# qingfengxia/FenicsSolver

Measured on AMD Instinct MI355X. Metric: DOF/s (assemble+CG solve to 1e-8) on 3D heat transfer, higher is better.
Workload: dtype f64

## Files before the change

fenicssolver_amd/csrc/fs_krylov.hip:

```cpp
#include "fs_common.h"
#include "fs_kernels.h"
#include <functional>
#include <chrono>
#include <string>
#include <unordered_map>
#include <math.h>
#include <stdlib.h>

#ifndef FS_BLOCK_ROUND
#define FS_BLOCK_ROUND 3
#endif

#include "fs_krylov_stream.inc"

#include "fs_krylov_dict.inc"

#define BOX_DC_AUX 2
#include "fs_box.h"
#include "fs_latmarch.h"
#include "fs_krylov_lattice.inc"

#include "fs_krylov_dict3.inc"

struct row_dict {
// ... 2058 lines not shown
                    hipLaunchKernelGGL(k_cg_update<true>, dim3(vgrid), dim3(FS_BLOCK), 0, s, n, k, k == max_iter ? 1 : 0, ws.partials.p, sgrid, ws.sums.p, ws.ctrl.p, ws.scal.p, ws.status.p, hist_p, ws.dinv.p, ws.z.p, ws.w.p, ws.p.p, ws.s.p, x->d.p, ws.r.p);
                } else {
                    FS_CHECK(fs_comm_sum_allreduce_dev(ws.partials.p, sgrid, 3, ws.sums.p, s));
                    if (sample) FS_HIP(hipEventRecord(ws.ev[n_samples][2], s));
                    hipLaunchKernelGGL(k_cg_update<false>, dim3(vgrid), dim3(FS_BLOCK), 0, s, n, k, k == max_iter ? 1 : 0, ws.partials.p, sgrid, ws.sums.p, ws.ctrl.p, ws.scal.p, ws.status.p, hist_p, ws.dinv.p, ws.z.p, ws.w.p, ws.p.p, ws.s.p, x->d.p, ws.r.p);
                }
                if (sample) {
                    FS_HIP(hipEventRecord(ws.ev[n_samples][3], s));
                    ++n_samples;
                }
            }
            FS_KERNEL_CHECK();
            n_launches += k - k_before;
            if (!mirrored) {
                FS_HIP(hipMemcpyAsync(ws.h_status + 4 * slot, ws.status.p, 4 * sizeof(int), hipMemcpyDeviceToHost, s));
                FS_HIP(hipEventRecord(ws.poll[slot], s));
                if (pending >= 0) {
                    FS_HIP(hipEventSynchronize(ws.poll[pending]));
                    if (ws.h_status[4 * pending] != 0) finished = true;
                }
                pending = slot;
                slot ^= 1;
            }
            if (k > max_iter) finished = true;
        }
        lap("iterations of the pass");
        if (sp->halo.begun) {
            FS_CHECK(fs_halo_end_dev(sp, s));
            sp->halo.begun = false;
        }
        if (red_stream) FS_HIP(hipStreamWaitEvent(s, ws.ev_red, 0));
        if (iteration_form & 1) {
            hipLaunchKernelGGL(k_cg_pair_flush, dim3(fs_grid_for(n / 2 + 1, FS_BLOCK, 2048)), dim3(FS_BLOCK), 0, s, n, ws.status.p, ws.scal.p, ws.z.p, ws.p.p, x->d.p);
            FS_KERNEL_CHECK();
        }
        FS_HIP(hipMemcpyAsync(ws.z.p, x->d.p, (size_t)n * sizeof(double), hipMemcpyDeviceToDevice, s));
        FS_CHECK(fs_halo_exchange_dev(sp, ws.z.p, s));
        launch_spmv<0>(A, ws.z.p, ws.w.p, nullptr, nullptr, nullptr, s, aval);
        if (ds) hipLaunchKernelGGL(k_residual_scaled, dim3(pgrid), dim3(FS_BLOCK), 0, s, ws.bhat.p, ws.w.p, ws.dvec.p, n, (double*)nullptr, ws.partials.p);
        else hipLaunchKernelGGL(k_residual, dim3(pgrid), dim3(FS_BLOCK), 0, s, b->d.p, ws.w.p, n, (double*)nullptr, ws.partials.p);
        FS_CHECK(fs_comm_sum_allreduce_dev(ws.partials.p, pgrid, 1, ws.sums.p + 5, s));
        FS_HIP(hipMemcpyAsync(ws.h_status + 12, ws.status.p, 4 * sizeof(int), hipMemcpyDeviceToHost, s));
        FS_HIP(hipMemcpyAsync(ws.h_vals, ws.sums.p, 8 * sizeof(double), hipMemcpyDeviceToHost, s));
        FS_HIP(hipMemcpyAsync(ws.h_vals + 8, ws.ctrl.p, 4 * sizeof(double), hipMemcpyDeviceToHost, s));
        FS_HIP(hipStreamSynchronize(s));
        if (fs_p2p_reduce_enabled()) FS_CHECK(fs_p2p_check(s));
        for (int q = 0; q < 4; ++q) h_status[q] = ws.h_status[12 + q];
        const int iters = h_status[1];
        total_iters += iters;
        for (int i = first_sample; i < n_samples; ++i) ws.sample_live[i] = ws.sample_iter[i] + ws.sample_span[i] - 1 < iters;
        if (ws.h_status[8] != 0) {
            fs_set_error("fs_krylov_solve: %d zero%s diagonal entries (Jacobi preconditioner undefined)", ws.h_status[8], ds ? " or negative" : "");
            return FS_ERR_NUMERIC;
        }
        const double* h_pass = ws.h_vals;
        const double* h_ctrl2 = ws.h_vals + 8;
        true_rr = h_pass[5];
        thresh = h_ctrl2[0];
        bb_host = h_ctrl2[1];
        ++n_pass;
        if (getenv("FS_KRYLOV_DEBUG"))
            fprintf(stderr, "[fs_krylov] pass %d: status %d, %d iterations (total %d), true ||r||^2 %.3e, threshold %.3e\n",
                    n_pass, h_status[0], h_status[1], total_iters, true_rr, thresh);
        const bool recurrence_converged = h_status[0] == 1;
        if (!recurrence_converged || true_rr <= thresh * 1.0201 || n_pass >= 8 || total_iters >= opts->max_iter) break;
        if (true_rr > 0.7 * prev_true_rr) break;
        prev_true_rr = true_rr;
        use_guess = true;
    }
    if (ds) {
        hipLaunchKernelGGL(k_pointwise_mul, dim3(fs_grid_for(n)), dim3(FS_BLOCK), 0, s, ws.dinv.p, x->d.p, n, x->d.p);
        FS_KERNEL_CHECK();
    }
    const int iters = total_iters;
    if (fs_rt().comm && getenv("FS_COMM_TIMING")) {
        double au, hu; long ac, hc;
        fs_comm_host_time(&au, &ac, &hu, &hc, true);
        fprintf(stderr, "[fs_krylov] host time inside RCCL enqueue calls: all-reduce %.1f us x %ld, grouped send/recv %.1f us x %ld; %d iterations in %.1f ms\n",
                ac ? au / ac : 0.0, ac, hc ? hu / hc : 0.0, hc, iters,
                std::chrono::duration<double, std::milli>(std::chrono::steady_clock::now() - t_begin).count());
    }
#ifdef FS_ITER_TIMING
    if (fused && getenv("FS_ITER_TIMING")) {
        std::vector<long long> h(8 * 4096);
        FS_HIP(hipMemcpyFromSymbol(h.data(), HIP_SYMBOL(g_iter_dbg), h.size() * sizeof(long long)));
        long long first = h[0], last = 0;
        for (int b = 0; b < igrid; ++b) { first = std::min(first, h[8 * b]); last = std::max(last, h[8 * b + 7]); }
        double mean[8] = {0}, mx[8] = {0};
        for (int b = 0; b < igrid; ++b)
            for (int k2 = 0; k2 < 8; ++k2) { const double v = (h[8 * b + k2] - first) * 0.01; mean[k2] += v / igrid; mx[k2] = std::max(mx[k2], v); }
        fprintf(stderr, "[iter timing, last launch, us from the first workgroup's start] span %.2f;", (last - first) * 0.01);
        for (int k2 = 0; k2 < 8; ++k2) fprintf(stderr, " s%d mean %.2f max %.2f;", k2, mean[k2], mx[k2]);
        fprintf(stderr, "\n");
        std::vector<int32_t> hi((size_t)sp->n_dict_items * 4);
        FS_CHECK(sp->dict_items.download(hi.data(), (int64_t)hi.size(), s));
        FS_HIP(hipStreamSynchronize(s));
        const int64_t n_chunks = (sp->n_dict_items + 3) / 4, per_xcd = (n_chunks + 7) >> 3;
        int cnt[2] = {0, 0};
        double gm[2][3] = {{0}}, gx[2][3] = {{0}};
        for (int b = 0; b < igrid; ++b) {
            int64_t cur = b, step = igrid, end = n_chunks;
            if (dict_map_xcd()) { cur = (b & 7) * per_xcd + (b >> 3); step = igrid >> 3; end = std::min<int64_t>(((b & 7) + 1) * per_xcd, n_chunks); }
            int e = 0;
            for (; cur < end; cur += step)
                for (int64_t q = 4 * cur; q < std::min<int64_t>(4 * cur + 4, sp->n_dict_items); ++q) e |= (hi[(size_t)q * 4 + 1] >> 16) & 1;
            ++cnt[e];
            for (int k2 = 0; k2 < 3; ++k2) { const double v = (h[8 * b + 5 + k2] - first) * 0.01; gm[e][k2] += v; gx[e][k2] = std::max(gx[e][k2], v); }
        }
        for (int e = 0; e < 2; ++e) {
            fprintf(stderr, "[iter timing] %d workgroups %s an edge item:", cnt[e], e ? "with" : "without");
            for (int k2 = 0; k2 < 3; ++k2) fprintf(stderr, " s%d mean %.2f max %.2f;", 5 + k2, cnt[e] ? gm[e][k2] / cnt[e] : 0.0, gx[e][k2]);
            fprintf(stderr, "\n");
        }
    }
#endif
    ws.last_hist.resize((size_t)iters + 1);
    FS_CHECK(ws.hist.download(ws.last_hist.data(), iters + 1, s));
    const auto t_end = std::chrono::steady_clock::now();

    if (stats) {
        memset(stats, 0, sizeof(*stats));
        const double bb = bb_host;
        stats->iterations = iters;
        stats->converged = h_status[0] == 2 ? -1 : (h_status[0] == 1 ? 1 : 0);
        stats->bnorm = sqrt(bb);
        stats->rel_residual = bb > 0.0 ? sqrt(ws.last_hist[iters] / bb) : 0.0;
        stats->true_rel_residual = bb > 0.0 ? sqrt(true_rr / bb) : sqrt(true_rr);
        stats->solve_ms = std::chrono::duration<double, std::milli>(t_end - t_begin).count();
        double t_spmv = 0.0, t_upd = 0.0;
        int cnt = 0;
        for (int i = 0; i < n_samples; ++i) {
            if (!ws.sample_live[i]) continue;
            float a = 0.f, c = 0.f;
            if (hipEventElapsedTime(&a, ws.ev[i][0], ws.ev[i][1]) != hipSuccess) break;
            if (hipEventElapsedTime(&c, ws.ev[i][2], ws.ev[i][3]) != hipSuccess) break;
            t_spmv += a / (float)ws.sample_span[i];
            t_upd += c;
            ++cnt;
        }
        if (cnt) {
            stats->spmv_ms = t_spmv / cnt;
            stats->update_ms = t_upd / cnt;
        }
        stats->spmv_bytes = sp->nnz_nodes * bs * bs * 12 + n * 20;
        stats->row_classes = g_dict.built_for ? g_dict.ncls : 0;
        stats->fused_iteration = fusedp_used ? 2 : (fused ? 1 : 0);
        stats->classes_kept = g_dict.built_for && g_dict.kept ? 1 : 0;
        stats->launches = n_launches;
        stats->product_kind = fused ? (BI ? 3 : 1) : g_last_product_kind;
        g_last_iteration_form = (fused || fusedp_used) ? iteration_form : 0;
        if (fused) stats->update_ms = 0.0;
    }
    if (h_status[0] == 2) {
        fs_set_error("fs_krylov_solve: %s breakdown at iteration %d (operator not SPD / rho = 0 / NaN)", bicg ? "BiCGStab" : "CG", iters);
        return FS_ERR_NUMERIC;
    }
    return FS_OK;
}

extern "C" int fs_last_iteration_form() { return g_last_iteration_form & 3; }
extern "C" int fs_last_iteration_guard() { return (g_last_iteration_form >> 2) & 3; }
void fs_krylov_set_history(const std::vector<double>& rr) { g_ws.last_hist = rr; }
void fs_set_last_product_kind(int kind) { g_last_product_kind = kind; }

extern "C" int fs_krylov_history(double* out, int capacity, int* count) {
    const int n = (int)g_ws.last_hist.size();
    if (count) *count = n;
    if (out)
        for (int i = 0; i < n && i < capacity; ++i) out[i] = g_ws.last_hist[i];
    return FS_OK;
}

void fs_krylov_preload() {
    hipFuncAttributes attr;
    (void)hipFuncGetAttributes(&attr, reinterpret_cast<const void*>(k_set_threshold));
    (void)hipGetLastError();
}
```

fenicssolver_amd/csrc/fs_krylov_dict.inc:

```

constexpr int FS_DICT_CAP = 8192;
constexpr int FS_DICT_MAX = 4096;
constexpr int FS_DICT_ITEM_ROWS = 126;
constexpr int FS_DICT_WHOLE_LDS_BYTES = 32 << 10;
constexpr int FS_DICT_LDS_BYTES = 64 << 10;
constexpr int FS_DICT_ITEMS_PER_WAVE = 4;
constexpr int FS_DICT3_RUNS = 4;
constexpr int FS_DICT_MAX_ROUNDS = 8;

struct dict_plan_round {
    int32_t start[8];
    uint8_t len[8];
    uint8_t pad[24];
};
static_assert(sizeof(dict_plan_round) == 64, "one 64-byte scalar load per round");
struct dict_plan_round12 {
    int32_t start[12];
    uint8_t len[12];
    uint8_t pad[4];
};
static_assert(sizeof(dict_plan_round12) == 64, "one 64-byte scalar load per round");
__host__ __device__ __forceinline__ int32_t dict_run_start(const dict_plan_round* __restrict__ pl, int NR, int g) {
    return reinterpret_cast<const int32_t*>(pl + g / NR)[g % NR];
}
// ... 207 lines not shown
            if (slot_d) dtab[id] = slot_d[slot];
        }
        id += used;
    }
}

__global__ void __launch_bounds__(FS_BLOCK) k_dict_finish(int64_t n_items, const int4* __restrict__ items, const dict_plan_round* __restrict__ plans,
                                                          const int64_t* __restrict__ slice_ptr, const int32_t* __restrict__ dia_ptr,
                                                          const int32_t* __restrict__ dia_off, const double* __restrict__ val, int nq, int64_t plane, int S, int RL,
                                                          const int32_t* __restrict__ slot2cls, const double* __restrict__ values,
                                                          const int32_t* __restrict__ nnz, const uint16_t* __restrict__ cls_slot,
                                                          uint16_t* __restrict__ cls, int* info, const double* __restrict__ sc = nullptr, int NR = 8,
                                                          const double* __restrict__ dvec = nullptr, const double* __restrict__ dtab = nullptr) {
    const int lane = threadIdx.x & 63;
    int64_t q = ((int64_t)blockIdx.x * blockDim.x + threadIdx.x) >> 6;
    const int64_t stride = ((int64_t)gridDim.x * blockDim.x) >> 6;
    int bad = 0, bad_d = 0, crowded = 0;
    for (; q < n_items; q += stride) {
        const int4 it = items[q];
        const int32_t first = it.x, nr = it.y & 0xffff;
        const dict_plan_round* __restrict__ pl = plans + it.z;
        const int n_runs = NR * it.w;
        int id2[2] = {-1, -1};
        for (int half = 0; half < 2; ++half) {
            const int i = half * 64 + lane;
            if (i >= nr) continue;
            const int32_t r = first + i;
            const int id = slot2cls[cls_slot[r]];
            cls[r] = (uint16_t)(id < 0 ? 0 : id);
            if (id < 0 || id >= FS_DICT_MAX) { ++bad; continue; }
            id2[half] = id;
            if (dvec) bad_d += __double_as_longlong(dvec[r]) != __double_as_longlong(dtab[id]);
            const double* __restrict__ dv = values + (int64_t)id * S;
            int nz = 0, diff = 0;
            const bool fits = dict_walk_row(r, slice_ptr, dia_ptr, dia_off, val, nq, plane, pl, n_runs, RL, [&](int slot, double v) {
                ++nz;
                diff += slot >= S || __double_as_longlong(v) != __double_as_longlong(dv[slot < S ? slot : 0]);
            }, sc, NR);
            bad += !fits || diff != 0 || nz != nnz[id];
        }
        int distinct = 0;
        unsigned long long m0 = __ballot(id2[0] >= 0), m1 = __ballot(id2[1] >= 0);
        while (m0 | m1) {
            const bool from0 = m0 != 0ull;
            const int src = __ffsll((long long)(from0 ? m0 : m1)) - 1;
            const int cv = __shfl(from0 ? id2[0] : id2[1], src, 64);
            m0 &= ~__ballot(id2[0] == cv);
            m1 &= ~__ballot(id2[1] == cv);
            ++distinct;
        }
        crowded = distinct > crowded ? distinct : crowded;
    }
    if (bad) atomicAdd(&info[2], bad);
    if (bad_d) atomicAdd(&info[4], bad_d);
    if (crowded && lane == 0 && crowded > __hip_atomic_load(&info[3], __ATOMIC_RELAXED, __HIP_MEMORY_SCOPE_AGENT)) atomicMax(&info[3], crowded);
}

__device__ __forceinline__ double fs_from_next_lane(double v) {
    const int lo = __builtin_amdgcn_update_dpp(0, __double2loint(v), 0x130, 0xf, 0xf, true);
    const int hi = __builtin_amdgcn_update_dpp(0, __double2hiint(v), 0x130, 0xf, 0xf, true);
    return __hiloint2double(hi, lo);
}

__device__ __forceinline__ void fs_fill_lds(double* __restrict__ lds, const double* __restrict__ g, int n) {
    typedef double v2d __attribute__((ext_vector_type(2)));
    const int n2 = n >> 1;
    const v2d* __restrict__ g2 = reinterpret_cast<const v2d*>(g);
    v2d* __restrict__ l2 = reinterpret_cast<v2d*>(lds);
    for (int base = 0; base < n2; base += 4 * FS_BLOCK) {
        v2d t[4];
#pragma unroll
        for (int u = 0; u < 4; ++u) {
            const int i = base + u * FS_BLOCK + (int)threadIdx.x;
            t[u] = g2[i < n2 ? i : n2 - 1];
        }
#pragma unroll
        for (int u = 0; u < 4; ++u) {
            const int i = base + u * FS_BLOCK + (int)threadIdx.x;
            if (i < n2) l2[i] = t[u];
        }
    }
}

__device__ __forceinline__ void fs_wave_copy_pairs(double* __restrict__ lds, const double* __restrict__ g, int n2, int lane) {
    typedef double v2d __attribute__((ext_vector_type(2)));
    const v2d* __restrict__ g2 = reinterpret_cast<const v2d*>(g);
    v2d* __restrict__ l2 = reinterpret_cast<v2d*>(lds);
    for (int base = 0; base < n2; base += 256) {
        v2d t[4];
#pragma unroll
        for (int u = 0; u < 4; ++u) {
            const int i = base + u * 64 + lane;
            t[u] = g2[i < n2 ? i : n2 - 1];
        }
#pragma unroll
        for (int u = 0; u < 4; ++u) {
            const int i = base + u * 64 + lane;
            if (i < n2) l2[i] = t[u];
        }
    }
}

template <int DOTS, bool LDSD, int RL, int NR = 8>
__global__ void __launch_bounds__(FS_BLOCK) k_dict_spmv(int64_t n_cols, int64_t n_items, const int4* __restrict__ items,
                                                        const dict_plan_round* __restrict__ plans, const uint16_t* __restrict__ cls,
                                                        const double* __restrict__ dict, int S, int C,
                                                        const double* __restrict__ x, double* __restrict__ y,
                                                        const double* __restrict__ rvec, double* __restrict__ partials,
                                                        int* __restrict__ status, int part_base, int part_stride, int bump, int map_xcd) {
    const int st0 = DOTS ? status[0] : 0;
    typedef double v2d __attribute__((ext_vector_type(2)));
    typedef double v2du __attribute__((ext_vector_type(2), aligned(8)));
    extern __shared__ __attribute__((aligned(16))) double sdict[];
    __shared__ double lds4[4];
    const int lane = threadIdx.x & 63;
    const int wave = threadIdx.x >> 6;
    double* __restrict__ wl = LDSD ? sdict : sdict + (int64_t)wave * C * S;
    if (LDSD) fs_fill_lds(sdict, dict, C * S);
    if (DOTS) {
        if (st0 != 0) return;
        if (bump && blockIdx.x == 0 && threadIdx.x == 0) status[2] += 1;
    }
    if (LDSD) __syncthreads();
    double d_rz = 0.0, d_wz = 0.0, d_rr = 0.0;
    constexpr int K = LDSD ? 1 : FS_DICT_ITEMS_PER_WAVE;
    const int64_t n_chunks = (n_items + 4 * K - 1) / (4 * K);
    const int32_t cmax = (int32_t)(n_cols - 1);
    chunk_iter it = xcd_chunks(n_chunks);
    if (!map_xcd) { it.cur = blockIdx.x; it.step = gridDim.x; it.end = n_chunks; }
    int tagv = -1, rr = 0;
    const unsigned long long cmask = C >= 64 ? ~0ull : ((1ull << C) - 1ull);
    for (; it.cur < it.end; it.cur += it.step)
    for (int kk = 0; kk < K; ++kk) {
        const int64_t q = (it.cur * 4 + wave) * K + kk;
        if (q >= n_items) break;
        const int4 ds = items[__builtin_amdgcn_readfirstlane((int)q)];
        const int32_t first = __builtin_amdgcn_readfirstlane(ds.x);
        const int nr = __builtin_amdgcn_readfirstlane(ds.y) & 0xffff;
        const int edge = __builtin_amdgcn_readfirstlane(ds.y) >> 16;
        const dict_plan_round* __restrict__ pl = plans + __builtin_amdgcn_readfirstlane(ds.z);
        const int rounds = __builtin_amdgcn_readfirstlane(ds.w);
        const int32_t r = first + 2 * lane;
        const bool ok0 = 2 * lane < nr, ok1 = 2 * lane + 1 < nr;
        v2d ri = {0.0, 0.0};
        if (DOTS && DOTS != 4) {
            if (ok1) ri = *reinterpret_cast<const v2du*>(&rvec[r]);
            else if (ok0) ri.x = rvec[r];
        }
        int c0 = -1, c1 = -1;
        if ((first & 1) == 0) {
            const uint32_t two = *reinterpret_cast<const uint32_t*>(&cls[r]);
            if (ok0) c0 = (int)(two & 0xffffu);
            if (ok1) c1 = (int)(two >> 16);
        } else {
            if (ok0) c0 = (int)cls[r];
            if (ok1) c1 = (int)cls[r + 1];
        }
        const double* __restrict__ xr = x + r;
        v2d A[NR];
        struct starts8 { int32_t v[NR]; };
        auto read_starts = [&](const dict_plan_round* __restrict__ p) {
            starts8 t;
#pragma unroll
            for (int j = 0; j < NR; ++j) t.v[j] = __builtin_amdgcn_readfirstlane(reinterpret_cast<const int32_t*>(p)[j]);
            return t;
        };
// ... 111 lines not shown
```

fenicssolver_amd/csrc/fs_krylov_iter.inc:

```

__global__ void k_set_threshold(const double* __restrict__ bb, double rtol, double atol, double* __restrict__ ctrl) {
    if (threadIdx.x == 0 && blockIdx.x == 0) {
        const double t = rtol * rtol * bb[0];
        ctrl[0] = fmax(t, atol * atol);
        ctrl[1] = bb[0];
    }
}
__global__ void k_set_iteration_limit(double* __restrict__ ctrl, int max_iter) {
    if (threadIdx.x == 0 && blockIdx.x == 0) ctrl[2] = (double)max_iter;
}

__device__ __forceinline__ bool cg_scalars_from(int iter, double gamma, double delta, double rho, double gamma_old, double alpha_old,
                                                 double& alpha, double& beta) {
    beta = 0.0;
    if (iter == 0) {
        alpha = gamma / delta;
    } else {
        beta = gamma / gamma_old;
        alpha = gamma / (delta - beta * gamma / alpha_old);
    }
    return (alpha > 0.0) && (alpha < 1e300) && (rho == rho);
}
__device__ __forceinline__ bool cg_scalars(int iter, double gamma, double delta, double rho, const double* __restrict__ scal,
                                            double& alpha, double& beta) {
// ... 285 lines not shown
    const bool first_trip = i + stride < n2;
    double2 wa0 = {0.0, 0.0}, wb0 = wa0, pa0 = wa0, sa0 = wa0, xa0 = wa0, ra0 = wa0, pb0 = wa0, sb0 = wa0, xb0 = wa0, rb0 = wa0;
    if (first_trip) {
        const int64_t j = i + stride;
        wa0 = io::ld(&w2[i]); wb0 = io::ld(&w2[j]);
        pa0 = io::ld(&p2[i]); sa0 = io::ld(&s2[i]); xa0 = io::ld(&x2[i]); ra0 = io::ld(&r2[i]);
        pb0 = io::ld(&p2[j]); sb0 = io::ld(&s2[j]); xb0 = io::ld(&x2[j]); rb0 = io::ld(&r2[j]);
    }
    if (st0 != 0) return;
    if (iter < 0) {
        iter = st2 - 1;
        check_only = iter >= (int)it_max ? 1 : 0;
    }
    double gamma, delta, rho;
    if (FUSED) {
        double sm[3];
        wg_sum_partials<3>(partials, npart, sm);
        gamma = sm[0]; delta = sm[1]; rho = sm[2];
    } else {
        gamma = sums[0]; delta = sums[1]; rho = sums[2];
    }
    const bool leader = blockIdx.x == 0 && threadIdx.x == 0;
    if (leader) hist[iter] = rho;
    auto stop = [&](int code) {
        if (leader) {
            status[1] = iter; status[0] = code;
            if (mirror) { fs_host_store(mirror + 1, iter); fs_host_store(mirror, code); }
        }
    };
    if (rho <= thresh) { stop(1); return; }
    if (check_only) { stop(3); return; }
    double beta, alpha;
    if (!cg_scalars_from(iter, gamma, delta, rho, ((iter - 1) & 1) ? sc_g1 : sc_g0, ((iter - 1) & 1) ? sc_a1 : sc_a0, alpha, beta)) { stop(2); return; }
    if (leader) {
        scal[2 * (iter & 1) + 0] = gamma;
        scal[2 * (iter & 1) + 1] = alpha;
        if (mirror) fs_host_store(mirror + 1, iter + 1);
    }
    bool prefetched = first_trip;
    for (; i + stride < n2; i += 2 * stride) {
        const int64_t j = i + stride;
        double2 wa, wb, pa, sa, xa, ra, pb, sb, xb, rb;
        if (prefetched) {
            wa = wa0; wb = wb0; pa = pa0; sa = sa0; xa = xa0; ra = ra0; pb = pb0; sb = sb0; xb = xb0; rb = rb0;
            prefetched = false;
        } else {
            wa = io::ld(&w2[i]); wb = io::ld(&w2[j]);
            pa = io::ld(&p2[i]); sa = io::ld(&s2[i]); xa = io::ld(&x2[i]); ra = io::ld(&r2[i]);
            pb = io::ld(&p2[j]); sb = io::ld(&s2[j]); xb = io::ld(&x2[j]); rb = io::ld(&r2[j]);
        }
        pa.x = ra.x + beta * pa.x;  pa.y = ra.y + beta * pa.y;
        pb.x = rb.x + beta * pb.x;  pb.y = rb.y + beta * pb.y;
        sa.x = wa.x + beta * sa.x;  sa.y = wa.y + beta * sa.y;
        sb.x = wb.x + beta * sb.x;  sb.y = wb.y + beta * sb.y;
        xa.x += alpha * pa.x;       xa.y += alpha * pa.y;
        xb.x += alpha * pb.x;       xb.y += alpha * pb.y;
        ra.x -= alpha * sa.x;       ra.y -= alpha * sa.y;
        rb.x -= alpha * sb.x;       rb.y -= alpha * sb.y;
        if (r_plain & 2) { p2[i] = pa; p2[j] = pb; } else { io::st(&p2[i], pa); io::st(&p2[j], pb); }
        if (r_plain & 4) { s2[i] = sa; s2[j] = sb; } else { io::st(&s2[i], sa); io::st(&s2[j], sb); }
        if (r_plain & 8) { x2[i] = xa; x2[j] = xb; } else { io::st(&x2[i], xa); io::st(&x2[j], xb); }
        if (r_plain & 1) { r2[i] = ra; r2[j] = rb; } else { io::st(&r2[i], ra); io::st(&r2[j], rb); }
    }
    for (; i < n2; i += stride) {
        const double2 ww = w2[i];
        double2 pp = p2[i], ss = s2[i], xx = x2[i], rr = r2[i];
        pp.x = rr.x + beta * pp.x;  pp.y = rr.y + beta * pp.y;
        ss.x = ww.x + beta * ss.x;  ss.y = ww.y + beta * ss.y;
        xx.x += alpha * pp.x;       xx.y += alpha * pp.y;
        rr.x -= alpha * ss.x;       rr.y -= alpha * ss.y;
        p2[i] = pp; s2[i] = ss; x2[i] = xx; r2[i] = rr;
    }
    if ((n & 1) && blockIdx.x == 0 && threadIdx.x == 0) {
        const int64_t t = n - 1;
        const double pp = r[t] + beta * p[t];
        const double ss = w[t] + beta * sv[t];
        p[t] = pp; sv[t] = ss;
        x[t] += alpha * pp;
        r[t] -= alpha * ss;
    }
}

#ifdef FS_ITER_TIMING
__device__ long long g_iter_dbg[8 * 4096];
#define FS_STAMP(k) do { if (threadIdx.x == 0 && it_ctr[par] == 100) g_iter_dbg[8 * blockIdx.x + (k)] = wall_clock64(); } while (0)
#else
#define FS_STAMP(k) do { } while (0)
#endif
enum { FS_ITER_EVERY = 0, FS_ITER_LIGHT = 1, FS_ITER_PAIR = 2 };
template <int RL, bool COMM, int MODE = FS_ITER_EVERY, bool DTAB = false, bool GUARD = false, bool CENTRE = false>
__global__ void __launch_bounds__(FS_BLOCK) k_dict_cg_iter(int64_t n_cols, int64_t n_items, const int4* __restrict__ items,
                                                           const dict_plan_round* __restrict__ plans, const uint16_t* __restrict__ cls,
                                                           const double* __restrict__ dict, int S, int C,
                                                           const double* __restrict__ r_in, const double* __restrict__ w_in,
                                                           const double* __restrict__ s_in, double* __restrict__ r_out,
                                                           double* __restrict__ w_out, double* __restrict__ s_out,
                                                           double* __restrict__ pv, double* __restrict__ xv, const double* __restrict__ dvec,
                                                           const double* __restrict__ part_in, double* __restrict__ part_out, int npart,
                                                           const double* __restrict__ ctrl, double* __restrict__ scal, int* __restrict__ status,
                                                           int* __restrict__ it_ctr, int par, double* __restrict__ hist, int map_xcd,
                                                           const double* __restrict__ sums, int* __restrict__ mirror) {
    FS_STAMP(0);
    const int st0 = status[0];
    const int iter = it_ctr[par];
    const double thresh = ctrl[0], it_max = ctrl[2];
    const double sc_g0 = scal[0], sc_a0 = scal[1], sc_g1 = scal[2], sc_a1 = scal[3];
    double sc_b0 = 0.0, sc_b1 = 0.0;
    if (MODE == FS_ITER_PAIR) { sc_b0 = scal[4]; sc_b1 = scal[5]; }
    double dt0 = 0.0;
    if (DTAB) dt0 = dvec[(int)threadIdx.x < C ? (int)threadIdx.x : 0];
    double pl[3][4];
    double sum_g = 0.0, sum_d = 0.0, sum_r = 0.0;
    if (COMM) { sum_g = sums[0]; sum_d = sums[1]; sum_r = sums[2]; }
    else {
#pragma unroll
        for (int t = 0; t < 4; ++t) {
            const int i = threadIdx.x + t * FS_BLOCK;
#pragma unroll
            for (int j = 0; j < 3; ++j) pl[j][t] = part_in[(int64_t)j * npart + (i < npart ? i : npart - 1)];
        }
    }
    FS_STAMP(1);
    typedef double v2d __attribute__((ext_vector_type(2)));
    typedef double v2du __attribute__((ext_vector_type(2), aligned(8)));
    extern __shared__ __attribute__((aligned(16))) double sdict[];
    __shared__ double lds34[3][4];
    const int lane = threadIdx.x & 63;
    const int wave = threadIdx.x >> 6;
    const int64_t n_chunks = (n_items + 3) / 4;
    const int32_t cmax = (int32_t)(n_cols - 1);
    chunk_iter it = xcd_chunks(n_chunks);
    if (!map_xcd) { it.cur = blockIdx.x; it.step = gridDim.x; it.end = n_chunks; }
    struct item_hdr { int32_t first; int nr, edge, rounds; const dict_plan_round* pl; };
    auto decode = [&](int64_t q) {
        const int4 ds = items[__builtin_amdgcn_readfirstlane((int)q)];
        item_hdr H;
        H.first = __builtin_amdgcn_readfirstlane(ds.x);
        H.nr = __builtin_amdgcn_readfirstlane(ds.y) & 0xffff;
        H.edge = __builtin_amdgcn_readfirstlane(ds.y) >> 16;
        H.pl = plans + __builtin_amdgcn_readfirstlane(ds.z);
        H.rounds = __builtin_amdgcn_readfirstlane(ds.w);
        return H;
    };
    auto load_half = [&](const item_hdr& H, int rd, int h, uint32_t boff, v2d (&A)[4], v2d (&Wb)[4], v2d (&Sb)[4], bool skip0 = false) {
        int32_t sts[4];
#pragma unroll
        for (int j = 0; j < 4; ++j) sts[j] = __builtin_amdgcn_readfirstlane(H.pl[rd].start[4 * h + j]);
#pragma unroll
        for (int j = 0; j < 4; ++j) {
            if (skip0 && j == 0) { A[0] = Wb[0] = Sb[0] = v2d{0.0, 0.0}; continue; }
            const int32_t st = sts[j];
            A[j] = *reinterpret_cast<const v2du*>(reinterpret_cast<const char*>(r_in + st) + boff);
            Wb[j] = *reinterpret_cast<const v2du*>(reinterpret_cast<const char*>(w_in + st) + boff);
            Sb[j] = *reinterpret_cast<const v2du*>(reinterpret_cast<const char*>(s_in + st) + boff);
        }
    };
    auto load_own = [&](const item_hdr& H, v2d& pp, v2d& xx, v2d& dd, v2d& rp) {
        const int32_t r = H.first + 2 * lane;
        pp = xx = dd = rp = v2d{0.0, 0.0};
#ifdef FS_ITER_ABLATE_PXD
        dd = v2d{1.0, 1.0};
        return;
#endif
        if (2 * lane + 1 < H.nr) {
            if (MODE != FS_ITER_LIGHT) {
                pp = *reinterpret_cast<const v2du*>(&pv[r]);
                xx = *reinterpret_cast<const v2du*>(&xv[r]);
            }
            if (MODE == FS_ITER_PAIR) rp = *reinterpret_cast<const v2du*>(&r_out[r]);
            if (!DTAB) dd = *reinterpret_cast<const v2du*>(&dvec[r]);
        } else if (2 * lane < H.nr) {
            if (MODE != FS_ITER_LIGHT) { pp.x = pv[r]; xx.x = xv[r]; }
            if (MODE == FS_ITER_PAIR) rp.x = r_out[r];
            if (!DTAB) dd.x = dvec[r];
        }
    };
    item_hdr H0 = {};
    v2d PA[4], PW[4], PS[4], Ppp = {0.0, 0.0}, Pxx = {0.0, 0.0}, Pdd = {0.0, 0.0}, Prp = {0.0, 0.0};
    const bool have0 = it.cur < it.end && it.cur * 4 + wave < n_items;
    if (have0) {
        H0 = decode(it.cur * 4 + wave);
        if (GUARD || !H0.edge) load_half(H0, 0, 0, (uint32_t)(H0.first + 2 * lane) * 8u, PA, PW, PS, CENTRE);
        load_own(H0, Ppp, Pxx, Pdd, Prp);
    }
    FS_STAMP(2);
    fs_fill_lds(sdict, dict, C * S);
    double* const sdtab = sdict + C * S;
    if (DTAB) {
        if ((int)threadIdx.x < C) sdtab[threadIdx.x] = dt0;
        for (int i = (int)threadIdx.x + FS_BLOCK; i < C; i += FS_BLOCK) sdtab[i] = dvec[i];
    }
    if (st0 != 0) return;
    double sm[3];
    if (COMM) {
        sm[0] = sum_g; sm[1] = sum_d; sm[2] = sum_r;
        __syncthreads();
    } else {
        double a[3] = {0.0, 0.0, 0.0};
#pragma unroll
        for (int t = 0; t < 4; ++t)
            if ((int)threadIdx.x + t * FS_BLOCK < npart) {
#pragma unroll
                for (int j = 0; j < 3; ++j) a[j] += pl[j][t];
            }
#pragma unroll
        for (int j = 0; j < 3; ++j) {
#pragma unroll
            for (int off = 32; off > 0; off >>= 1) a[j] += __shfl_down(a[j], off, 64);
            if (lane == 0) lds34[j][wave] = a[j];
        }
        __syncthreads();
#pragma unroll
        for (int j = 0; j < 3; ++j) sm[j] = (lds34[j][0] + lds34[j][1]) + (lds34[j][2] + lds34[j][3]);
        __syncthreads();
    }
    FS_STAMP(3);
    const double gamma = sm[0], delta = sm[1], rho = sm[2];
    const bool leader = blockIdx.x == 0 && threadIdx.x == 0;
    if (leader) hist[iter] = rho;
    auto stop = [&](int code) {
        if (leader) {
            status[1] = iter; status[0] = code;
            if (mirror) { fs_host_store(mirror + 1, iter); fs_host_store(mirror, code); }
        }
    };
    if (rho <= thresh) { stop(1); return; }
    if (iter >= (int)it_max) { stop(3); return; }
    double beta, alpha;
    if (!cg_scalars_from(iter, gamma, delta, rho, ((iter - 1) & 1) ? sc_g1 : sc_g0, ((iter - 1) & 1) ? sc_a1 : sc_a0, alpha, beta)) { stop(2); return; }
    if (leader) {
        scal[2 * (iter & 1) + 0] = gamma;
        scal[2 * (iter & 1) + 1] = alpha;
        if (MODE != FS_ITER_EVERY) scal[4 + (iter & 1)] = beta;
        it_ctr[par ^ 1] = iter + 1;
        if (mirror) fs_host_store(mirror + 1, iter + 1);
    }
    const double nalpha = -alpha;
    const double alpha_prev = ((iter - 1) & 1) ? sc_a1 : sc_a0, beta_prev = ((iter - 1) & 1) ? sc_b1 : sc_b0;
    FS_STAMP(4);
    double d_rz = 0.0, d_wz = 0.0, d_rr = 0.0;
    auto do_item = [&](const item_hdr& H, auto pre_tag) {
        constexpr bool PRE = decltype(pre_tag)::value;
        const int32_t r = H.first + 2 * lane;
        const bool ok0 = 2 * lane < H.nr, ok1 = 2 * lane + 1 < H.nr;
        int c0 = -1, c1 = -1;
        if ((H.first & 1) == 0) {
            const uint32_t two = *reinterpret_cast<const uint32_t*>(&cls[r]);
            if (ok0) c0 = (int)(two & 0xffffu);
            if (ok1) c1 = (int)(two >> 16);
        } else {
            if (ok0) c0 = (int)cls[r];
            if (ok1) c1 = (int)cls[r + 1];
        }
        v2d sn0 = {0.0, 0.0}, ro0 = {0.0, 0.0};
        v2d pp, xx, dd, rp;
        if (PRE) { pp = Ppp; xx = Pxx; dd = Pdd; rp = Prp; }
        else load_own(H, pp, xx, dd, rp);
        if (DTAB) { dd.x = sdtab[ok0 ? c0 : 0]; dd.y = sdtab[ok1 ? c1 : 0]; }
        const double* __restrict__ v0 = sdict + (ok0 ? c0 * S : 0);
        const double* __restrict__ v1 = sdict + (ok1 ? c1 * S : 0);
        double a0 = 0.0, a1 = 0.0;
        v2d zi = {0.0, 0.0};
        auto run_terms = [&](v2d rn, const double* __restrict__ w0, const double* __restrict__ w1) {
            const double e0 = rn.x, e1 = rn.y;
            const double e2 = fs_from_next_lane(rn.x);
            a0 = fma(w0[0], e0, a0); a1 = fma(w1[0], e1, a1);
            a0 = fma(w0[1], e1, a0); a1 = fma(w1[1], e2, a1);
            if (RL == 3) {
                const double e3 = fs_from_next_lane(rn.y);
                a0 = fma(w0[2], e2, a0); a1 = fma(w1[2], e3, a1);
            }
        };
        if (GUARD || !H.edge) {
            const uint32_t boff = (uint32_t)r * 8u;
            for (int rd = 0; rd < H.rounds; ++rd) {
#pragma unroll
                for (int h = 0; h < 2; ++h) {
                    v2d A[4], Wb[4], Sb[4];
                    const bool skip0 = CENTRE && h == 0;
                    if (PRE && h == 0) {
                        if (rd == 0) {
#pragma unroll
                            for (int j = 0; j < 4; ++j) { A[j] = PA[j]; Wb[j] = PW[j]; Sb[j] = PS[j]; }
                        } else load_half(H, rd, h, boff, A, Wb, Sb);
                    } else load_half(H, rd, h, boff, A, Wb, Sb, skip0);
#pragma unroll
                    for (int j = 0; j < 4; ++j) {
                        if (skip0 && j == 0) continue;
                        v2d sn;
                        sn.x = fma(beta, Sb[j].x, Wb[j].x); sn.y = fma(beta, Sb[j].y, Wb[j].y);
                        if (!CENTRE && h == 0 && j == 0 && rd == 0) { sn0 = sn; ro0 = A[0]; }
                        if (CENTRE && h == 1 && j == 0) {
                            sn0.x = sn.y; sn0.y = fs_from_next_lane(sn.x);
                            ro0.x = A[0].y; ro0.y = fs_from_next_lane(A[0].x);
                        }
                        A[j].x = fma(nalpha, sn.x, A[j].x); A[j].y = fma(nalpha, sn.y, A[j].y);
                    }
                    if (!CENTRE && h == 0 && rd == 0) zi = A[0];
                    if (CENTRE && h == 1) { zi.x = A[0].y; zi.y = fs_from_next_lane(A[0].x); }
#pragma unroll
                    for (int j = 0; j < 4; ++j) {
                        if (skip0 && j == 0) continue;
                        run_terms(A[j], v0 + RL * (8 * rd + 4 * h + j), v1 + RL * (8 * rd + 4 * h + j));
                        asm volatile("" ::: "memory");
                    }
                }
            }
        } else {
            const int n_runs = 8 * H.rounds;
#pragma unroll 1
            for (int g = 0; g < n_runs; ++g) {
                const int32_t c = r + __builtin_amdgcn_readfirstlane(H.pl[g >> 3].start[g & 7]);
                const int32_t ca = c < 0 ? 0 : (c > cmax ? cmax : c), cb = c + 1 < 0 ? 0 : (c + 1 > cmax ? cmax : c + 1);
                v2d rn, sn;
                sn.x = fma(beta, s_in[ca], w_in[ca]); sn.y = fma(beta, s_in[cb], w_in[cb]);
                const double ra = r_in[ca], rb = r_in[cb];
                if (g == 0) { sn0 = sn; ro0.x = ra; ro0.y = rb; }
                rn.x = fma(nalpha, sn.x, ra); rn.y = fma(nalpha, sn.y, rb);
                if (g == 0) zi = rn;
                run_terms(rn, v0 + RL * g, v1 + RL * g);
            }
        }
        v2d pn = {0.0, 0.0}, xn = {0.0, 0.0};
        if (MODE == FS_ITER_PAIR) {
            pp.x = fma(beta_prev, pp.x, rp.x); pp.y = fma(beta_prev, pp.y, rp.y);
            xx.x = fma(alpha_prev, pp.x, xx.x); xx.y = fma(alpha_prev, pp.y, xx.y);
        }
        if (MODE != FS_ITER_LIGHT) {
            pn.x = fma(beta, pp.x, ro0.x); pn.y = fma(beta, pp.y, ro0.y);
            xn.x = fma(alpha, pn.x, xx.x); xn.y = fma(alpha, pn.y, xx.y);
        }
        constexpr bool PX =
#ifdef FS_ITER_ABLATE_PXD
            false;
#else
            MODE != FS_ITER_LIGHT;
#endif
        if (ok1) {
            v2d out;
            out.x = a0; out.y = a1;
            *reinterpret_cast<v2du*>(&w_out[r]) = out;
            *reinterpret_cast<v2du*>(&r_out[r]) = zi;
            *reinterpret_cast<v2du*>(&s_out[r]) = sn0;
            if (PX) {
                *reinterpret_cast<v2du*>(&pv[r]) = pn;
                *reinterpret_cast<v2du*>(&xv[r]) = xn;
            }
        } else if (ok0) {
            w_out[r] = a0; r_out[r] = zi.x; s_out[r] = sn0.x;
            if (PX) { pv[r] = pn.x; xv[r] = xn.x; }
        }
        if (!ok0) { a0 = 0.0; zi.x = 0.0; }
        if (!ok1) { a1 = 0.0; zi.y = 0.0; }
        d_rz += zi.x * zi.x + zi.y * zi.y; d_wz += a0 * zi.x + a1 * zi.y; d_rr += dd.x * zi.x * zi.x + dd.y * zi.y * zi.y;
    };
    if (have0) {
        do_item(H0, std::true_type{});
        it.cur += it.step;
    }
    FS_STAMP(5);
    for (; it.cur < it.end; it.cur += it.step) {
        const int64_t q = it.cur * 4 + wave;
        if (q >= n_items) break;
        do_item(decode(q), std::false_type{});
    }
    FS_STAMP(6);
    double dsum[3] = {d_rz, d_wz, d_rr};
#pragma unroll
    for (int j = 0; j < 3; ++j) {
#pragma unroll
        for (int off = 32; off > 0; off >>= 1) dsum[j] += __shfl_down(dsum[j], off, 64);
        if (lane == 0) lds34[j][wave] = dsum[j];
    }
    __syncthreads();
    FS_STAMP(7);
    if (threadIdx.x < 3) part_out[(int64_t)threadIdx.x * npart + blockIdx.x] =
        (lds34[threadIdx.x][0] + lds34[threadIdx.x][1]) + (lds34[threadIdx.x][2] + lds34[threadIdx.x][3]);
}

__global__ void __launch_bounds__(FS_BLOCK) k_cg_pair_flush(int64_t n, const int* __restrict__ status, const double* __restrict__ scal,
                                                            const double* __restrict__ r_prev, const double* __restrict__ p, double* __restrict__ x) {
    const int st0 = status[0], it = status[1];
    const double alpha = scal[1], beta = scal[4];
    if (st0 == 0 || !(it & 1)) return;
    const int64_t n2 = n >> 1;
    const double2* __restrict__ r2 = reinterpret_cast<const double2*>(r_prev);
    const double2* __restrict__ p2 = reinterpret_cast<const double2*>(p);
    double2* __restrict__ x2 = reinterpret_cast<double2*>(x);
    const int64_t stride = (int64_t)gridDim.x * blockDim.x;
    for (int64_t i = (int64_t)blockIdx.x * blockDim.x + threadIdx.x; i < n2; i += stride) {
        const double2 rr = r2[i], pp = p2[i];
        double2 xx = x2[i];
        xx.x = fma(alpha, fma(beta, pp.x, rr.x), xx.x);
        xx.y = fma(alpha, fma(beta, pp.y, rr.y), xx.y);
        x2[i] = xx;
    }
    if ((n & 1) && blockIdx.x == 0 && threadIdx.x == 0) x[n - 1] = fma(alpha, fma(beta, p[n - 1], r_prev[n - 1]), x[n - 1]);
}

__global__ void __launch_bounds__(FS_BLOCK) k_cg_update_scaled_rows(int64_t a, int64_t b, int64_t n, int iter, int check_only,
                                                                    const double* __restrict__ sums, const double* __restrict__ ctrl,
                                                                    const double* __restrict__ scal, const int* __restrict__ status,
                                                                    double* __restrict__ r, const double* __restrict__ w,
                                                                    double* __restrict__ p, double* __restrict__ sv, double* __restrict__ x) {
    if (status[0] != 0) return;
    const double gamma = sums[0], delta = sums[1], rho = sums[2];
    if (rho <= ctrl[0] || check_only) return;
    double beta, alpha;
    if (!cg_scalars(iter, gamma, delta, rho, scal, alpha, beta)) return;
    const int64_t total = a + (n - b);
    int64_t t = (int64_t)blockIdx.x * blockDim.x + threadIdx.x;
    const int64_t stride = (int64_t)gridDim.x * blockDim.x;
    for (; t < total; t += stride) {
        const int64_t i = t < a ? t : b + (t - a);
        const double pp = r[i] + beta * p[i];
        const double ss = w[i] + beta * sv[i];
        p[i] = pp; sv[i] = ss;
        x[i] += alpha * pp;
        r[i] -= alpha * ss;
    }
}

struct fs_pp_ghosts {
    double* w_cur;
    const double* s_cur;
    double* s_nxt;
    const double* r_cur;
    double* r_nxt;
    const int* it_ctr;
    int par;
};
template <bool PP>
__global__ void __launch_bounds__(FS_BLOCK) k_cg_p2p_exchange(int iter, int check_only, const double* __restrict__ ctrl,
                                                              const double* __restrict__ scal, const int* __restrict__ status,
                                                              double* r, const double* __restrict__ w, double* __restrict__ s_ghost,
                                                              const fs_p2p_rowsred red, const fs_p2p_sendrows snd, const fs_pp_ghosts pp) {
    const int st0 = status[0], st2 = status[2];
    const double it_max = ctrl[2], thresh = ctrl[0];
    const double sc_g0 = scal[0], sc_a0 = scal[1], sc_g1 = scal[2], sc_a1 = scal[3];
    const unsigned long long rseq = *red.d_seq + 1ull, hseq = *snd.d_seq + 1ull;
    const int it_dev = PP ? pp.it_ctr[pp.par] : 0;
    if (st0 != 0) return;
    if (PP) {
        iter = it_dev;
        check_only = iter >= (int)it_max ? 1 : 0;
    } else if (iter < 0) {
        iter = st2 - 1;
        check_only = iter >= (int)it_max ? 1 : 0;
    }
    const int rslot = (int)(rseq & 1ull), hslot = (int)(hseq & 1ull);
    const int64_t e_first = (int64_t)blockIdx.x * blockDim.x + threadIdx.x;
    const int64_t stride = (int64_t)gridDim.x * blockDim.x;
    const int t = threadIdx.x;
    for (int64_t e = e_first; e < snd.total_send; e += stride) {
        const double wv = w[snd.send_idx[e]];
        int j = 0;
        while (j + 1 < snd.nn && e >= snd.peers[j + 1].send_offset) ++j;
        const fs_p2p_peer q = snd.peers[j];
        fs_p2p_store(q.recv + (int64_t)hslot * q.peer_total + q.recv_offset + (e - q.send_offset), wv);
    }
// ... 310 lines not shown
```

Measured before the change: 173.0 million.

## Issue async global-to-LDS dictionary fill at kernel entry and overlap with prologue loads

The dictionary and diagonal table are now copied into LDS with global_load_lds instructions issued at the very start of the fused CG iteration kernel, and explicit vmcnt waits are placed just before the barrier that needs them. The first item's operand loads are issued unconditionally in guarded mode through address-space-1 pointers, so they overlap the partial-sum reduction. A second LDS scratch array removes one barrier after the reduction. This targets the latency of the kernel prologue per CG iteration, at the cost of hand-counted waitcnt values that are fragile if the instruction mix changes. The timing stamps are also widened to 16 slots.

```diff
diff --git a/fenicssolver_amd/csrc/fs_krylov.hip b/fenicssolver_amd/csrc/fs_krylov.hip
--- a/fenicssolver_amd/csrc/fs_krylov.hip
+++ b/fenicssolver_amd/csrc/fs_krylov.hip
@@ -2164,15 +2164,15 @@
     }
 #ifdef FS_ITER_TIMING
     if (fused && getenv("FS_ITER_TIMING")) {
-        std::vector<long long> h(8 * 4096);
+        std::vector<long long> h(FS_STAMPS * 4096);
         FS_HIP(hipMemcpyFromSymbol(h.data(), HIP_SYMBOL(g_iter_dbg), h.size() * sizeof(long long)));
         long long first = h[0], last = 0;
-        for (int b = 0; b < igrid; ++b) { first = std::min(first, h[8 * b]); last = std::max(last, h[8 * b + 7]); }
-        double mean[8] = {0}, mx[8] = {0};
+        for (int b = 0; b < igrid; ++b) { first = std::min(first, h[FS_STAMPS * b]); last = std::max(last, h[FS_STAMPS * b + 7]); }
+        double mean[9] = {0}, mx[9] = {0};
         for (int b = 0; b < igrid; ++b)
-            for (int k2 = 0; k2 < 8; ++k2) { const double v = (h[8 * b + k2] - first) * 0.01; mean[k2] += v / igrid; mx[k2] = std::max(mx[k2], v); }
+            for (int k2 = 0; k2 < 9; ++k2) { const double v = (h[FS_STAMPS * b + k2] - first) * 0.01; mean[k2] += v / igrid; mx[k2] = std::max(mx[k2], v); }
         fprintf(stderr, "[iter timing, last launch, us from the first workgroup's start] span %.2f;", (last - first) * 0.01);
-        for (int k2 = 0; k2 < 8; ++k2) fprintf(stderr, " s%d mean %.2f max %.2f;", k2, mean[k2], mx[k2]);
+        for (int k2 = 0; k2 < 9; ++k2) fprintf(stderr, " s%d mean %.2f max %.2f;", k2, mean[k2], mx[k2]);
         fprintf(stderr, "\n");
         std::vector<int32_t> hi((size_t)sp->n_dict_items * 4);
         FS_CHECK(sp->dict_items.download(hi.data(), (int64_t)hi.size(), s));
@@ -2187,7 +2187,7 @@
             for (; cur < end; cur += step)
                 for (int64_t q = 4 * cur; q < std::min<int64_t>(4 * cur + 4, sp->n_dict_items); ++q) e |= (hi[(size_t)q * 4 + 1] >> 16) & 1;
             ++cnt[e];
-            for (int k2 = 0; k2 < 3; ++k2) { const double v = (h[8 * b + 5 + k2] - first) * 0.01; gm[e][k2] += v; gx[e][k2] = std::max(gx[e][k2], v); }
+            for (int k2 = 0; k2 < 3; ++k2) { const double v = (h[FS_STAMPS * b + 5 + k2] - first) * 0.01; gm[e][k2] += v; gx[e][k2] = std::max(gx[e][k2], v); }
         }
         for (int e = 0; e < 2; ++e) {
             fprintf(stderr, "[iter timing] %d workgroups %s an edge item:", cnt[e], e ? "with" : "without");
diff --git a/fenicssolver_amd/csrc/fs_krylov_dict.inc b/fenicssolver_amd/csrc/fs_krylov_dict.inc
--- a/fenicssolver_amd/csrc/fs_krylov_dict.inc
+++ b/fenicssolver_amd/csrc/fs_krylov_dict.inc
@@ -313,6 +313,28 @@
     }
 }
 
+template <int B = 16>
+__device__ __forceinline__ void fs_fill_lds_issue(double* lds, const double* __restrict__ g, int n) {
+    static_assert(B == 16 || B == 4, "dwordx4 or dword");
+    const int nc = B == 16 ? n >> 1 : 2 * n;
+    const int lane = threadIdx.x & 63;
+    const int w64 = __builtin_amdgcn_readfirstlane((int)threadIdx.x & ~63);
+    const char* g8 = reinterpret_cast<const char*>(g);
+    char* l8 = reinterpret_cast<char*>(lds);
+    for (int base = w64; base < nc; base += FS_BLOCK)
+        if (base + lane < nc) {
+            const auto* src = (const __attribute__((address_space(1))) void*)(g8 + (int64_t)(base + lane) * B);
+            auto* dst = (__attribute__((address_space(3))) void*)(l8 + base * B);
+            if (B == 16) __builtin_amdgcn_global_load_lds(src, dst, 16, 0, 0);
+            else __builtin_amdgcn_global_load_lds(src, dst, 4, 0, 0);
+        }
+    __builtin_amdgcn_sched_barrier(0);
+}
+template <int AFTER>
+__device__ __forceinline__ void fs_fill_lds_wait() {
+    asm volatile("s_waitcnt vmcnt(%0)" ::"n"(AFTER) : "memory");
+}
+
 __device__ __forceinline__ void fs_wave_copy_pairs(double* __restrict__ lds, const double* __restrict__ g, int n2, int lane) {
     typedef double v2d __attribute__((ext_vector_type(2)));
     const v2d* __restrict__ g2 = reinterpret_cast<const v2d*>(g);
diff --git a/fenicssolver_amd/csrc/fs_krylov_iter.inc b/fenicssolver_amd/csrc/fs_krylov_iter.inc
--- a/fenicssolver_amd/csrc/fs_krylov_iter.inc
+++ b/fenicssolver_amd/csrc/fs_krylov_iter.inc
@@ -391,12 +391,21 @@
 }
 
 #ifdef FS_ITER_TIMING
-__device__ long long g_iter_dbg[8 * 4096];
-#define FS_STAMP(k) do { if (threadIdx.x == 0 && it_ctr[par] == 100) g_iter_dbg[8 * blockIdx.x + (k)] = wall_clock64(); } while (0)
+#define FS_STAMPS 16
+__device__ long long g_iter_dbg[FS_STAMPS * 4096];
+#define FS_STAMP(k) do { if (threadIdx.x == 0 && it_ctr[par] == 100) g_iter_dbg[FS_STAMPS * blockIdx.x + (k)] = wall_clock64(); } while (0)
 #else
 #define FS_STAMP(k) do { } while (0)
 #endif
 enum { FS_ITER_EVERY = 0, FS_ITER_LIGHT = 1, FS_ITER_PAIR = 2 };
+typedef const __attribute__((address_space(1))) double* fs_gcd;
+typedef double fs_v2du __attribute__((ext_vector_type(2), aligned(8)));
+__device__ __forceinline__ fs_v2du fs_ld_pair(const double* base, int32_t st, uint32_t boff) {
+    return *reinterpret_cast<const fs_v2du*>(reinterpret_cast<const char*>(base + st) + boff);
+}
+__device__ __forceinline__ fs_v2du fs_ld_pair(fs_gcd base, int32_t st, uint32_t boff) {
+    return *(const __attribute__((address_space(1))) fs_v2du*)((const __attribute__((address_space(1))) char*)(base + st) + boff);
+}
 template <int RL, bool COMM, int MODE = FS_ITER_EVERY, bool DTAB = false, bool GUARD = false, bool CENTRE = false>
 __global__ void __launch_bounds__(FS_BLOCK) k_dict_cg_iter(int64_t n_cols, int64_t n_items, const int4* __restrict__ items,
                                                            const dict_plan_round* __restrict__ plans, const uint16_t* __restrict__ cls,
@@ -410,14 +419,18 @@
                                                            int* __restrict__ it_ctr, int par, double* __restrict__ hist, int map_xcd,
                                                            const double* __restrict__ sums, int* __restrict__ mirror) {
     FS_STAMP(0);
+    extern __shared__ __attribute__((aligned(16))) double sdict[];
+    fs_fill_lds_issue(sdict, dict, C * S);
+    double* const sdtab = sdict + C * S;
+    if (DTAB) fs_fill_lds_issue<4>(sdtab, dvec, C);
     const int st0 = status[0];
     const int iter = it_ctr[par];
     const double thresh = ctrl[0], it_max = ctrl[2];
     const double sc_g0 = scal[0], sc_a0 = scal[1], sc_g1 = scal[2], sc_a1 = scal[3];
     double sc_b0 = 0.0, sc_b1 = 0.0;
     if (MODE == FS_ITER_PAIR) { sc_b0 = scal[4]; sc_b1 = scal[5]; }
-    double dt0 = 0.0;
-    if (DTAB) dt0 = dvec[(int)threadIdx.x < C ? (int)threadIdx.x : 0];
+    fs_gcd part_pre = (fs_gcd)part_in, r_pre = (fs_gcd)r_in, w_pre = (fs_gcd)w_in, s_pre = (fs_gcd)s_in;
+    asm volatile("" : "+s"(part_pre), "+s"(r_pre), "+s"(w_pre), "+s"(s_pre));
     double pl[3][4];
     double sum_g = 0.0, sum_d = 0.0, sum_r = 0.0;
     if (COMM) { sum_g = sums[0]; sum_d = sums[1]; sum_r = sums[2]; }
@@ -426,14 +439,13 @@
         for (int t = 0; t < 4; ++t) {
             const int i = threadIdx.x + t * FS_BLOCK;
 #pragma unroll
-            for (int j = 0; j < 3; ++j) pl[j][t] = part_in[(int64_t)j * npart + (i < npart ? i : npart - 1)];
+            for (int j = 0; j < 3; ++j) pl[j][t] = part_pre[(int64_t)j * npart + (i < npart ? i : npart - 1)];
         }
     }
     FS_STAMP(1);
     typedef double v2d __attribute__((ext_vector_type(2)));
     typedef double v2du __attribute__((ext_vector_type(2), aligned(8)));
-    extern __shared__ __attribute__((aligned(16))) double sdict[];
-    __shared__ double lds34[3][4];
+    __shared__ double lds34[3][4], lds34e[3][4];
     const int lane = threadIdx.x & 63;
     const int wave = threadIdx.x >> 6;
     const int64_t n_chunks = (n_items + 3) / 4;
@@ -451,7 +463,7 @@
         H.rounds = __builtin_amdgcn_readfirstlane(ds.w);
         return H;
     };
-    auto load_half = [&](const item_hdr& H, int rd, int h, uint32_t boff, v2d (&A)[4], v2d (&Wb)[4], v2d (&Sb)[4], bool skip0 = false) {
+    auto load_half = [&](const item_hdr& H, int rd, int h, uint32_t boff, v2d (&A)[4], v2d (&Wb)[4], v2d (&Sb)[4], bool skip0 = false, bool pre = false) {
         int32_t sts[4];
 #pragma unroll
         for (int j = 0; j < 4; ++j) sts[j] = __builtin_amdgcn_readfirstlane(H.pl[rd].start[4 * h + j]);
@@ -459,9 +471,8 @@
         for (int j = 0; j < 4; ++j) {
             if (skip0 && j == 0) { A[0] = Wb[0] = Sb[0] = v2d{0.0, 0.0}; continue; }
             const int32_t st = sts[j];
-            A[j] = *reinterpret_cast<const v2du*>(reinterpret_cast<const char*>(r_in + st) + boff);
-            Wb[j] = *reinterpret_cast<const v2du*>(reinterpret_cast<const char*>(w_in + st) + boff);
-            Sb[j] = *reinterpret_cast<const v2du*>(reinterpret_cast<const char*>(s_in + st) + boff);
+            if (pre) { A[j] = fs_ld_pair(r_pre, st, boff); Wb[j] = fs_ld_pair(w_pre, st, boff); Sb[j] = fs_ld_pair(s_pre, st, boff); }
+            else { A[j] = fs_ld_pair(r_in, st, boff); Wb[j] = fs_ld_pair(w_in, st, boff); Sb[j] = fs_ld_pair(s_in, st, boff); }
         }
     };
     auto load_own = [&](const item_hdr& H, v2d& pp, v2d& xx, v2d& dd, v2d& rp) {
@@ -484,25 +495,57 @@
             if (!DTAB) dd.x = dvec[r];
         }
     };
+    auto load_own_pre = [&](const item_hdr& H, bool have, v2d& pp, v2d& xx, v2d& dd, v2d& rp) {
+        const int32_t r = H.first + 2 * lane;
+        pp = xx = dd = rp = v2d{0.0, 0.0};
+#ifdef FS_ITER_ABLATE_PXD
+        dd = v2d{1.0, 1.0};
+        return;
+#endif
+        if (have && 2 * lane < H.nr) {
+            if (MODE != FS_ITER_LIGHT) { pp.x = pv[r]; xx.x = xv[r]; }
+            if (MODE == FS_ITER_PAIR) rp.x = r_out[r];
+            if (!DTAB) dd.x = dvec[r];
+        }
+        if (have && 2 * lane + 1 < H.nr) {
+            if (MODE != FS_ITER_LIGHT) { pp.y = pv[r + 1]; xx.y = xv[r + 1]; }
+            if (MODE == FS_ITER_PAIR) rp.y = r_out[r + 1];
+            if (!DTAB) dd.y = dvec[r + 1];
+        }
+    };
     item_hdr H0 = {};
     v2d PA[4], PW[4], PS[4], Ppp = {0.0, 0.0}, Pxx = {0.0, 0.0}, Pdd = {0.0, 0.0}, Prp = {0.0, 0.0};
     const bool have0 = it.cur < it.end && it.cur * 4 + wave < n_items;
-    if (have0) {
+    constexpr int RUN_LOADS0 = GUARD ? 3 * (CENTRE ? 3 : 4) : 0;
+    if (GUARD) {
+        H0 = decode(have0 ? it.cur * 4 + wave : 0);
+        load_own_pre(H0, have0, Ppp, Pxx, Pdd, Prp);
+        load_half(H0, 0, 0, (uint32_t)(H0.first + 2 * lane) * 8u, PA, PW, PS, CENTRE, true);
+    } else if (have0) {
         H0 = decode(it.cur * 4 + wave);
-        if (GUARD || !H0.edge) load_half(H0, 0, 0, (uint32_t)(H0.first + 2 * lane) * 8u, PA, PW, PS, CENTRE);
+        if (!H0.edge) load_half(H0, 0, 0, (uint32_t)(H0.first + 2 * lane) * 8u, PA, PW, PS, CENTRE, true);
         load_own(H0, Ppp, Pxx, Pdd, Prp);
     }
+    asm volatile("" ::: "memory");
     FS_STAMP(2);
-    fs_fill_lds(sdict, dict, C * S);
-    double* const sdtab = sdict + C * S;
-    if (DTAB) {
-        if ((int)threadIdx.x < C) sdtab[threadIdx.x] = dt0;
-        for (int i = (int)threadIdx.x + FS_BLOCK; i < C; i += FS_BLOCK) sdtab[i] = dvec[i];
-    }
-    if (st0 != 0) return;
+    if (st0 != 0) {
+        fs_fill_lds_wait<0>();
+        return;
+    }
+    FS_STAMP(8);
+    if (GUARD && !COMM) {
+        __builtin_amdgcn_s_waitcnt(0x0f70 | RUN_LOADS0);
+        asm volatile("s_nop 0");
+#pragma unroll
+        for (int t = 0; t < 4; ++t) {
+#pragma unroll
+            for (int j = 0; j < 3; ++j) asm volatile("" : "+v"(pl[j][t]));
+        }
+    }
     double sm[3];
     if (COMM) {
         sm[0] = sum_g; sm[1] = sum_d; sm[2] = sum_r;
+        fs_fill_lds_wait<0>();
         __syncthreads();
     } else {
         double a[3] = {0.0, 0.0, 0.0};
@@ -518,10 +561,10 @@
             for (int off = 32; off > 0; off >>= 1) a[j] += __shfl_down(a[j], off, 64);
             if (lane == 0) lds34[j][wave] = a[j];
         }
+        fs_fill_lds_wait<RUN_LOADS0>();
         __syncthreads();
 #pragma unroll
         for (int j = 0; j < 3; ++j) sm[j] = (lds34[j][0] + lds34[j][1]) + (lds34[j][2] + lds34[j][3]);
-        __syncthreads();
     }
     FS_STAMP(3);
     const double gamma = sm[0], delta = sm[1], rho = sm[2];
@@ -679,12 +722,12 @@
     for (int j = 0; j < 3; ++j) {
 #pragma unroll
         for (int off = 32; off > 0; off >>= 1) dsum[j] += __shfl_down(dsum[j], off, 64);
-        if (lane == 0) lds34[j][wave] = dsum[j];
+        if (lane == 0) lds34e[j][wave] = dsum[j];
     }
     __syncthreads();
     FS_STAMP(7);
     if (threadIdx.x < 3) part_out[(int64_t)threadIdx.x * npart + blockIdx.x] =
-        (lds34[threadIdx.x][0] + lds34[threadIdx.x][1]) + (lds34[threadIdx.x][2] + lds34[threadIdx.x][3]);
+        (lds34e[threadIdx.x][0] + lds34e[threadIdx.x][1]) + (lds34e[threadIdx.x][2] + lds34e[threadIdx.x][3]);
 }
 
 __global__ void __launch_bounds__(FS_BLOCK) k_cg_pair_flush(int64_t n, const int* __restrict__ status, const double* __restrict__ scal,
```

Measured after the change: 186.3 million (median of 6 runs). +7.7%, better.
